# DavidSevic/gpu-nbody-simulation

Measured on AMD Instinct MI355X. Metric: body-steps/sec, higher is better.
Workload: dtype f32

## Files before the change

### gpu-nbody-simulation_amd/csrc/bh_engine.hip

```cpp
#include "../../include/bhgpu.h"

#include <hip/hip_runtime.h>

#include <algorithm>
#include <cmath>
#include <cstdio>
#include <cstdlib>
#include <cstring>
#include <string>
#include <type_traits>
#include <vector>

#include "bh_tree.hpp"
#include "bh_walk_exact.hpp"
#include "bh_walk_f64.hpp"
#include "bh_diag.hpp"
#include "bh_direct.hpp"
#include "bh_field.hpp"
#include "bh_init.hpp"
#include "bh_let.hpp"
#include "bh_migrate.hpp"
#include "bh_split.hpp"
#include "bh_moments.hpp"
#include "bh_radial.hpp"
// ... 28 lines not shown
    double eps = 0.0, eps2 = 0.0;
    float eps2f = 0.f;
    bool exact_thresholds = false;
    int device = 0;
    hipStream_t stream = nullptr;
    bool own_stream = false;
    int64_t n = 0;
    int64_t internal_cap = 0, node_cap = 0;
    int64_t bfs_max = 12288;
    int exact_bpw = 0;
    int walk_split = 0;
    bool walk_asm = true;
    int sort_bucket = 1;
    uint64_t *splitters = nullptr;
    uint16_t *sort_dig = nullptr;
    int build_items = 0;
    bool hilbert = false;
    bool chain_collapse = true;
    double *bslots = nullptr;

    void *pos = nullptr, *vel = nullptr, *mass = nullptr, *force = nullptr;
    void *pos2 = nullptr, *vel2 = nullptr, *mass2 = nullptr, *force2 = nullptr;
    uint32_t *orig = nullptr, *orig2 = nullptr;
    int reorder_every = 16;
    float2 *spos = nullptr;
    float4 *sstate = nullptr;
    float *smass = nullptr;
    uint64_t *keys[2] = {nullptr, nullptr};
    uint32_t *vals[2] = {nullptr, nullptr};
    uint64_t *keys_sorted = nullptr;
// ... 213 lines not shown

void clean_slots(bh_ctx *c) { if (c->carry.slots_dirty) hipLaunchKernelGGL(bounds_slots_reset, dim3(1), dim3(kWave), 0, c->stream, c->bslots); }

template <int SI>
int enqueue_lsd_passes(hipStream_t st, uint64_t *const keys[2], uint32_t *const vals[2], uint32_t *counts, uint32_t *rows, int64_t n,
                       int bits, bool packed)
{
    constexpr int SB = kSortBits;
    const unsigned nbl = blocks_for(n, kBlock * SI);
    const int passes = (bits + SB - 1) / SB;
    int cur = 0;
    for (int p = 0; p < passes; ++p) {
        const int shift = p * SB;
        auto scatter = [&](auto kern) {
            hipLaunchKernelGGL(kern, dim3(nbl), dim3(kBlock), 0, st, keys[cur], packed ? nullptr : vals[cur], keys[cur ^ 1],
                               vals[cur ^ 1], counts, rows, n, shift, (int)nbl, nullptr, nullptr);
        };
        hipLaunchKernelGGL((radix_hist<SI, SB>), dim3(nbl), dim3(kBlock), 0, st, keys[cur], counts, n, shift, (int)nbl);
        hipLaunchKernelGGL(radix_rowscan, dim3(1 << SB), dim3(kBlock), 0, st, counts, rows, (int)nbl);
        if (!packed) scatter(radix_scatter_w<SI, SB>);
        else if (p + 1 == passes) scatter(radix_scatter_w<SI, SB, 2>);
        else scatter(radix_scatter_w<SI, SB, 1>);
        cur ^= 1;
    }
    return cur;
}

template <bool TREE64, bool STATE64 = TREE64, int ITEMS = kItems>
int enqueue_build_t(bh_ctx *c, bool may_reorder, bool time_groups)
{
    constexpr int TILE = kBlock * ITEMS;
// ... 15 lines not shown
            hipLaunchKernelGGL((bounds_partial<Real2>), dim3(nbb), dim3(kBlock), 0, st, pos, n, slots);
        }
    }
    BuildDone done{n, slots != nullptr, false, false, false, false};

    if (n > 0) {
        const bool pack = Dm >= 1 && 2 * Dm <= kPackShift && n <= ((int64_t)1 << (64 - kPackShift))
                          && c->sort_pack;
        const bool single = pack && n >= 2 && n <= 4 * kBsThreads && c->sort_bucket == 1;
        const bool bucket = !single && pack && n >= 2 && n <= kBucketMaxNBig && (c->sort_bucket == 2 || (c->sort_bucket == 1 && c->carry.samples_n == n));
        const int nb = (n <= kBucketMaxN) ? kBuckets : kBucketsBig;
        const int ns = (nb == kBuckets) ? ((n > (int64_t)1 << 18) ? 2 * kBuckets : kBuckets)
                                        : ((n > (int64_t)3 << 20) ? kMaxSplitSamples : kBucketsBig);
        static_assert(kBucketMaxN == (int64_t)1 << 20 && kBucketMaxNBig == (int64_t)1 << 22, "BASELINE configs 3 and 4 fit");
        done.sort_bucket = bucket || single; done.sort_packed = pack;
        {
            const unsigned nkb = blocks_for(n, kBlock);
            auto keys_launch = [&](auto fs, auto pk, auto hil) {
                constexpr bool H = decltype(hil)::value, P = decltype(pk)::value, F = decltype(fs)::value;
                const bool smp = P && bucket;
                hipLaunchKernelGGL((keys_kernel<Real2, H, P, F>), dim3(nkb + (smp ? ns / kWave : 0)), dim3(kBlock), 0, st, pos, c->box,
                                   c->keys[0], c->vals[0], n, Dm, (smp && !TREE64) ? (const float2 *)c->spos : nullptr, c->splitters, nb, ns,
                                   slots, c->ctr, smp ? c->bsum_sort : nullptr, smp ? nb : 0, (smp && TREE64) ? c->perm : nullptr,
                                   from_walk ? 1 : 0);
            };
            dispatch(keys_launch, slots != nullptr, pack, c->hilbert);
        }
        if (time_groups) (void)hipEventRecord(c->ev_grp[0], st);
        const unsigned nbl = blocks_for(n, ITEMS == kItems ? kSortTile : TILE);
        int cur = 0;
        if (single) {
            hipLaunchKernelGGL(bucket_sort_kernel, dim3(1), dim3(kBsThreads), 0, st, c->keys[0], c->keys[1], c->vals[1],
                               nullptr, nullptr, &c->ctr->sort_spills, &c->ctr->sort_reruns, (int)n);
            cur = 1;
        } else if (bucket) {
            constexpr int SI = (ITEMS == kItems ? kSortItems : ITEMS);
            auto pass = [&](auto bits_tag) {
                constexpr int NBITS = decltype(bits_tag)::value;
                if constexpr (TREE64) {
                    hipLaunchKernelGGL((radix_hist<SI, NBITS, true>), dim3(nbl), dim3(kBlock), 0, st, c->keys[0], c->radix_counts, n,
                                       0, (int)nbl, c->splitters, c->sort_dig, nullptr);
                    hipLaunchKernelGGL(radix_rowscan, dim3(1 << NBITS), dim3(kBlock), 0, st, c->radix_counts, c->bsum_sort, (int)nbl);
                    hipLaunchKernelGGL((radix_scatter_w<SI, NBITS, 1, true, false>), dim3(nbl), dim3(kBlock), 0, st, c->keys[0], c->vals[0],
                                       c->keys[1], c->vals[1], c->radix_counts, c->bsum_sort, n, 0, (int)nbl, c->sort_dig,
                                       c->bsum_sort + kBucketStartOffset);
                } else {
                    hipLaunchKernelGGL((radix_hist<SI, NBITS, true>), dim3(nbl), dim3(kBlock), 0, st, c->keys[0], c->radix_counts, n,
                                       0, (int)nbl, c->splitters, c->sort_dig, c->bsum_sort);
                    hipLaunchKernelGGL((radix_scatter_w<SI, NBITS, 1, true>), dim3(nbl), dim3(kBlock), 0, st, c->keys[0], c->vals[0],
                                       c->keys[1], c->vals[1], c->radix_counts, c->bsum_sort, n, 0, (int)nbl, c->sort_dig,
                                       c->bsum_sort + kBucketStartOffset);
                }
            };
            if (nb == kBuckets) pass(std::integral_constant<int, 8>{}); else pass(std::integral_constant<int, 10>{});
            hipLaunchKernelGGL(bucket_sort_kernel, dim3(nb), dim3(kBsThreads), 0, st, c->keys[1], c->keys[0], c->vals[0],
                               c->bsum_sort, c->bsum_sort + kBucketStartOffset, &c->ctr->sort_spills, &c->ctr->sort_reruns, 0);
            cur = 0;
        } else {
            constexpr int SI = (ITEMS == kItems ? kSortItems : ITEMS);
            cur = enqueue_lsd_passes<SI>(st, c->keys, c->vals, c->radix_counts, c->bsum_sort, n, 2 * Dm, pack);
        }
        c->keys_sorted = c->keys[cur];
        c->perm = c->vals[cur];
        if constexpr (!TREE64) {
            if (may_reorder && c->reorder_every > 0 && c->carry.builds % c->reorder_every == 0) {
                hipLaunchKernelGGL((reorder_state_kernel<Real2, Real>), dim3(blocks_for(n, kBlock)), dim3(kBlock), 0, st,
                                   c->perm, pos, static_cast<const Real2 *>(c->vel), mass,
                                   static_cast<const float2 *>(c->force), c->is.orig_identity ? nullptr : c->orig,
                                   static_cast<Real2 *>(c->pos2), static_cast<Real2 *>(c->vel2),
                                   static_cast<Real *>(c->mass2), static_cast<float2 *>(c->force2), c->orig2, n);
                std::swap(c->pos, c->pos2); std::swap(c->vel, c->vel2); std::swap(c->mass, c->mass2);
                std::swap(c->force, c->force2); std::swap(c->orig, c->orig2);
// ... 388 lines not shown
    bh_ctx *c = new bh_ctx();
    c->cfg = *cfg;
    c->Dm = cfg->max_depth - 1;
    c->mode = cfg->precision == BH_PRECISION_F64_EXACT ? Mode::Exact
            : cfg->precision == BH_PRECISION_F64       ? Mode::F64
            : cfg->precision == BH_PRECISION_MIXED     ? Mode::Mixed : Mode::F32;
    c->compat = cfg->reference_compat != 0;
    c->device = cfg->device;
    if (const char *e = std::getenv("BH_WALK_SPLIT")) c->walk_split = std::atoi(e);
    if (const char *e = std::getenv("BH_EXACT_BPW")) { const int b = std::atoi(e); c->exact_bpw = (b >= 1 && b <= kWave && (b & (b - 1)) == 0) ? b : 0; }
    if (const char *e = std::getenv("BH_WALK_ASM")) c->walk_asm = std::atoi(e) != 0;
    if (const char *e = std::getenv("BH_EXACT_BFS_MAX")) c->bfs_max = std::max(0, std::atoi(e));
    c->exact_thresholds = c->mode == Mode::Exact && c->walk_asm && !(cfg->flags & BH_FLAG_WALK_PORTABLE);
    if (const char *e = std::getenv("BH_SORT_PACK")) c->sort_pack = std::atoi(e) != 0;
    if (const char *e = std::getenv("BH_SORT_BUCKET")) c->sort_bucket = std::atoi(e);
    if (const char *e = std::getenv("BH_BUILD_ITEMS")) c->build_items = std::atoi(e);
    if (const char *e = std::getenv("BH_REORDER_EVERY")) c->reorder_every = std::max(0, std::atoi(e));
    c->hilbert = !c->tree64();
    if (const char *e = std::getenv("BH_HILBERT")) c->hilbert = !c->tree64() && std::atoi(e) != 0;
    if (const char *e = std::getenv("BH_CHAIN_COLLAPSE")) c->chain_collapse = std::atoi(e) != 0;
    if (const char *e = std::getenv("BH_RADIAL_BLOCKS")) { const int b = std::atoi(e); if (b >= 1 && b <= 65536) c->rad_blocks = b; }
    auto bail = [&](int rc) { g_create_error = c->err; bh_destroy(c); return rc; };

    if (hipSetDevice(c->device) != hipSuccess) { c->err = "hipSetDevice failed"; return bail(BH_ERR_DEVICE); }
    if (hipStreamCreateWithFlags(&c->stream, hipStreamNonBlocking) != hipSuccess) {
        c->err = "hipStreamCreate failed"; return bail(BH_ERR_DEVICE);
    }
    c->own_stream = true;

    const int64_t cap = std::max<int64_t>(cfg->capacity, 1);
// ... 15 lines not shown
    if (!c->tree64()) {
        { char *t; A(&t, cap * 2 * rs); c->pos2 = t; }
        { char *t; A(&t, cap * 2 * rs); c->vel2 = t; }
        { char *t; A(&t, cap * rs); c->mass2 = t; }
        { char *t; A(&t, cap * 2 * sizeof(float)); c->force2 = t; }
        A(&c->orig, cap); A(&c->orig2, cap);
    }
    A(&c->keys[0], cap); A(&c->keys[1], cap); A(&c->vals[0], cap); A(&c->vals[1], cap);
    A(&c->cnt, cap + 1);
    { const size_t nbl = std::max<size_t>(blocks_for(cap, kSortTile), blocks_for(std::min<int64_t>(cap, 1 << 22), kBlock * kSmallItems));
      const size_t big = (cap > kBucketMaxN) ? (size_t)kBucketsBig * blocks_for(std::min<int64_t>(cap, kBucketMaxNBig), kBlock * kSmallItems) : 0;
      A(&c->radix_counts, std::max<size_t>((size_t)(1 << kSortBits) * nbl, big));
      A(&c->bsum_sort, 2 * kBucketStartOffset);
      A(&c->splitters, kBucketsBig);
      A(&c->sort_dig, (size_t)std::min<int64_t>(cap, kBucketMaxNBig) + 16);
    }
    const size_t scan_tiles = std::max<size_t>(blocks_for(cap + 1, kTile), blocks_for(std::min<int64_t>(cap, 1 << 22) + 1, kBlock * kSmallItems)) + 8;
    A(&c->bsum_u32, scan_tiles);
    A(&c->partial, 4 * (std::max<size_t>(1024, blocks_for(cap, kWave)) + 2));
    A(&c->box, 8); A(&c->bslots, 4 * kBoundSlots);
    A(&c->ctr, 1);
    if (c->tree64()) {
        { NodeD *g0 = nullptr; LinkD *l0 = nullptr; A(&g0, c->node_cap + 4); A(&l0, c->node_cap + 4);
          if (!rc) { c->gd = g0 + 3; c->ld = l0 + 3; } }
        A(&c->self_node, c->internal_cap + 1); A(&c->com_pending, c->internal_cap + 1); A(&c->cell_depth, c->internal_cap + 1);
        A(&c->cell_first, c->internal_cap + 1);
    } else {
        A(&c->qf, c->internal_cap + 1); A(&c->aux, 4 * (c->internal_cap + 1));
        A(&c->cell_first, c->internal_cap + 1);
        A(&c->gid, cap); A(&c->group_cost, cap / kWave + 2); A(&c->walk_consts, 4);
        A(&c->coarse, cap / 256 + 2);
        A(&c->spos, cap); A(&c->sstate, cap + 64 * kBlock + 1024); A(&c->smass, cap);
        A(&c->terms, cap + 1); A(&c->bsum_d3, scan_tiles);
    }
    if (rc) return bail(rc);
    if (hipMemset(c->ctr, 0, sizeof(TreeCounters)) != hipSuccess) { c->err = "hipMemset failed"; return bail(BH_ERR_DEVICE); }
    if (!c->tree64()) {
        const void *wc[4] = {c->aux, c->spos, c->smass, nullptr};
        if (hipMemcpy(c->walk_consts, wc, sizeof(wc), hipMemcpyHostToDevice) != hipSuccess) { c->err = "hipMemcpy failed"; return bail(BH_ERR_DEVICE); }
    }
    if (!c->tree64() && c->exp.create(cap) != hipSuccess) { c->err = "experiment hooks: allocation failed"; return bail(BH_ERR_DEVICE); }
    auto create = [](auto &evs) { for (auto &e : evs) if (hipEventCreate(&e) != hipSuccess) return false; return true; };
    if (!create(c->ev_step) || !create(c->ev_build) || !create(c->ev_grp) || !create(c->ev_let)) {
        c->err = "hipEventCreate failed"; return bail(BH_ERR_DEVICE);
    }
    *out = c;
    return BH_OK;
}

void bh_destroy(bh_ctx *c)
{
// ... 2235 lines not shown
```

### gpu-nbody-simulation_amd/csrc/bh_sort.hpp

```cpp
#pragma once

#include "bh_prims.hpp"

namespace bh {

#ifndef BH_SORT_ITEMS
#define BH_SORT_ITEMS 8
#endif
constexpr int kSortItems = BH_SORT_ITEMS;
constexpr int kSortTile = kBlock * kSortItems;
constexpr int kRadixBits = 8;

__global__ __launch_bounds__(kBlock) void radix_rowscan(uint32_t *__restrict__ counts,
                                                         uint32_t *__restrict__ row_total, int nblocks)
{
    __shared__ uint32_t sm[kWavesPerBlock + 1];
    uint32_t *row = counts + (int64_t)blockIdx.x * nblocks;
    uint32_t carry = 0;
    for (int c0 = 0; c0 < nblocks; c0 += kBlock) {
        const int b = c0 + threadIdx.x;
        const uint32_t v = (b < nblocks) ? row[b] : 0u;
        uint32_t tot;
        const uint32_t ex = block_exclusive_sum(v, sm, tot);
        if (b < nblocks) row[b] = carry + ex;
// ... 8 lines not shown
constexpr int kSortBits = 8;
constexpr int kBuckets = 256, kBucketsBig = 1024;
constexpr int kBucketStartOffset = kBucketsBig + 8;
constexpr int kDigits = 256;
constexpr int kMaxSplitSamples = 2048;
constexpr uint64_t kKeyMask40 = (1ull << 40) - 1;
template <int NB>
__device__ __forceinline__ uint32_t bucket_of(uint64_t key, const uint64_t *spl)
{
    int b = 0;
#pragma unroll
    for (int s = NB / 2; s >= 1; s >>= 1) b += (spl[b + s] <= key) ? s : 0;
    return (uint32_t)b;
}

__device__ __forceinline__ bool wave_same_digit(uint32_t d, bool valid)
{
    return __ballot(valid) == ~0ull && __ballot(d != (uint32_t)__builtin_amdgcn_readfirstlane((int)d)) == 0ull;
}
template <bool TRY = true>
__device__ __forceinline__ void wave_count_digit(uint32_t *row, uint32_t d, bool valid)
{
    if (TRY && wave_same_digit(d, valid)) {
        if (lane_id() == 0) atomicAdd(&row[d], (uint32_t)kWave);
    } else if (valid) {
        atomicAdd(&row[d], 1u);
    }
}

template <int ITEMS, int BITS = kRadixBits, bool BUCKET = false>
__global__ __launch_bounds__(kBlock) void radix_hist(const uint64_t *__restrict__ keys,
                                                      uint32_t *__restrict__ counts, int64_t n,
                                                      int shift, int nblocks,
                                                      const uint64_t *__restrict__ splitters = nullptr,
                                                      uint16_t *__restrict__ dig16 = nullptr,
                                                      uint32_t *__restrict__ row_total = nullptr)
{
    constexpr int R = 1 << BITS;
    __shared__ uint32_t h[R];
    __shared__ uint64_t spl[BUCKET ? R : 1];
    if (BUCKET)
        for (int d = threadIdx.x; d < R; d += kBlock) {
            const uint64_t v = splitters[d];
            spl[d] = (d > 0 && splitters[d - 1] == v) ? v + 1 : v;
        }
    for (int d = threadIdx.x; d < R; d += kBlock) h[d] = 0;
    __syncthreads();
    const int64_t base = (int64_t)blockIdx.x * (kBlock * ITEMS);
    uint32_t guess = 0;
#pragma unroll
    for (int r = 0; r < ITEMS; ++r) {
        const int64_t i = base + r * kBlock + threadIdx.x;
        const bool valid = i < n;
        const uint64_t k = valid ? keys[i] : 0ull;
        uint32_t d;
        if (BUCKET) {
            const uint64_t kk = k & kKeyMask40;
            bool ok = false;
            if (r > 0) ok = spl[guess] <= kk && (guess + 1 == (uint32_t)R || kk < spl[guess + 1]);
            if (r > 0 && __ballot(valid && !ok) == 0ull) d = guess;
            else d = bucket_of<R>(kk, spl);
            guess = d;
// ... 11 lines not shown
    }
}


constexpr int kPackShift = 40;
constexpr uint64_t kPackKeyMask = (1ull << kPackShift) - 1;
template <int ITEMS, int BITS = kRadixBits, int PACK = 0, bool BUCKET = false, bool RAW = BUCKET>
__global__ __launch_bounds__(kBlock) void radix_scatter_w(const uint64_t *__restrict__ kin,
                                                           const uint32_t *__restrict__ vin,
                                                           uint64_t *__restrict__ kout,
                                                           uint32_t *__restrict__ vout,
                                                           const uint32_t *__restrict__ offs,
                                                           const uint32_t *__restrict__ row_total, int64_t n,
                                                           int shift, int nblocks,
                                                           const uint16_t *__restrict__ dig16 = nullptr,
                                                           uint32_t *__restrict__ bucket_start = nullptr)
{
    static_assert(!BUCKET || PACK == 1, "the bucket pass moves packed keys");
    constexpr int TILE = kBlock * ITEMS;
    constexpr int R = 1 << BITS, DPT = R / kBlock;
    static_assert(R % kBlock == 0, "whole digits per thread");
    __shared__ uint32_t woff[kWavesPerBlock][R];
    __shared__ int32_t gdelta[R];
    __shared__ uint64_t skey[TILE];
    __shared__ uint32_t sval[PACK ? 1 : TILE];
    __shared__ uint32_t sm[kWavesPerBlock + 1];
    __shared__ uint16_t sdig[BUCKET ? TILE : 1];
    __shared__ uint64_t match[kWavesPerBlock][R];
    constexpr int kRowsTogether = 64;
    __shared__ uint32_t s_np, s_plist[kRowsTogether], s_before[kRowsTogether];
    const int t = threadIdx.x, w = wave_id(), l = lane_id();
    for (int d = t; d < R; d += kBlock)
#pragma unroll
        for (int k = 0; k < kWavesPerBlock; ++k) { woff[k][d] = 0; match[k][d] = 0ull; }
    __syncthreads();

    const int64_t tile_base = (int64_t)blockIdx.x * TILE;
    const int64_t base = tile_base + (int64_t)w * (kWave * ITEMS);
    uint64_t key[ITEMS];
    uint32_t val[PACK ? 1 : ITEMS];
    uint32_t dig[ITEMS], rank[ITEMS], npeer[ITEMS];
#pragma unroll
    for (int r = 0; r < ITEMS; ++r) {
        const int64_t i = base + r * kWave + l;
        const bool valid = i < n;
        key[r] = valid ? kin[i] : ~0ull;
        if (!PACK) val[r] = valid ? vin[i] : 0u;
        dig[r] = BUCKET ? (valid ? (uint32_t)dig16[i] : 0u) : (uint32_t)(key[r] >> shift) & (R - 1);
    }
#pragma unroll
// ... 143 lines not shown
{
    const int w = wave_id();
    const uint32_t inc = wave_inclusive_sum(v);
    if (w < 4 && lane_id() == kWave - 1) sm[w] = inc;
    __syncthreads();
    uint32_t base = 0, tot = 0;
#pragma unroll
    for (int k = 0; k < 4; ++k) { const uint32_t q = sm[k]; base += (k < w) ? q : 0u; tot += q; }
    __syncthreads();
    total = tot;
    return base + inc - v;
}

constexpr int kFixRun = 8;
template <int ITEMS>
__device__ __forceinline__ void bucket_sort_lds(const uint64_t *__restrict__ in, int m, uint64_t *skey,
                                                uint32_t (*woff)[kDigits], uint64_t (*match)[kDigits],
                                                uint32_t *sm, uint64_t *s_red, uint32_t *s_flag,
                                                uint64_t *__restrict__ kout, uint32_t *__restrict__ vout,
                                                uint32_t *__restrict__ reruns)
{
    const int t = threadIdx.x, w = wave_id(), l = lane_id();
    const int wbase = w * (kWave * ITEMS);
    uint64_t key[ITEMS];
    uint64_t kmin = ~0ull, kmax = 0ull;
#pragma unroll
    for (int r = 0; r < ITEMS; ++r) {
        const int i = wbase + r * kWave + l;
        key[r] = (i < m) ? in[i] : ~0ull;
        if (i < m) {
            const uint64_t k = key[r] & kKeyMask40;
// ... 111 lines not shown
                    if ((q >> first) != top) break;
                    delta += ((q & lowmask) < low) ? 1 : 0;
                }
                too_long = too_long || (j < m && j - i > kFixRun);
                kout[i + delta] = kk + kmin;
                vout[i + delta] = (uint32_t)(word >> kPackShift);
            }
        }
        if (too_long) *s_flag = 1u;
        __syncthreads();
        if (*s_flag == 0u) return;
        if (t == 0) atomicAdd(reruns, 1u);
#pragma unroll
        for (int r = 0; r < ITEMS; ++r) {
            const int i = wbase + r * kWave + l;
            key[r] = (i < m) ? in[i] - kmin : ~0ull;
        }
        for (int k = t; k < kBsWaves * kDigits; k += kBsThreads) (&woff[0][0])[k] = 0;
        __syncthreads();
        first = 0; passes = full; fix = false;
    }
    for (int i = t; i < m; i += kBsThreads) {
        const uint64_t k = skey[i];
        kout[i] = (k & kKeyMask40) + kmin;
        vout[i] = (uint32_t)(k >> kPackShift);
    }
}

__global__ __launch_bounds__(kBsThreads) void bucket_sort_kernel(uint64_t *__restrict__ bucketed,
                                                                  uint64_t *__restrict__ kout,
                                                                  uint32_t *__restrict__ vout,
                                                                  const uint32_t *__restrict__ bucket_total,
                                                                  const uint32_t *__restrict__ bucket_start,
                                                                  uint32_t *__restrict__ spills,
                                                                  uint32_t *__restrict__ reruns, int single_m)
{
    __shared__ uint64_t skey[kBucketCap];
    __shared__ uint32_t woff[kBsWaves][kDigits];
    __shared__ uint64_t match[kBsWaves][kDigits];
    __shared__ uint32_t sm[8];
    __shared__ uint64_t s_or[2 * kBsWaves];
    __shared__ uint32_t s_flag;
    const int t = threadIdx.x, w = wave_id(), l = lane_id();
    const int64_t start = bucket_total ? (int64_t)bucket_start[blockIdx.x] : 0;
    const int m = bucket_total ? (int)bucket_total[blockIdx.x] : single_m;
    if (m == 0) return;
    uint64_t *in = bucketed + start;
    uint64_t *ko = kout + start;
    uint32_t *vo = vout + start;

    if (m <= 1 * kBsThreads) { bucket_sort_lds<1>(in, m, skey, woff, match, sm, s_or, &s_flag, ko, vo, reruns); return; }
    if (m <= 2 * kBsThreads) { bucket_sort_lds<2>(in, m, skey, woff, match, sm, s_or, &s_flag, ko, vo, reruns); return; }
    if (m <= 4 * kBsThreads) { bucket_sort_lds<4>(in, m, skey, woff, match, sm, s_or, &s_flag, ko, vo, reruns); return; }
    if (m <= 5 * kBsThreads) { bucket_sort_lds<5>(in, m, skey, woff, match, sm, s_or, &s_flag, ko, vo, reruns); return; }
    if (m <= 6 * kBsThreads) { bucket_sort_lds<6>(in, m, skey, woff, match, sm, s_or, &s_flag, ko, vo, reruns); return; }
    if (m <= 8 * kBsThreads) { bucket_sort_lds<8>(in, m, skey, woff, match, sm, s_or, &s_flag, ko, vo, reruns); return; }
    if (m <= kBucketCap) { bucket_sort_lds<kBucketItemsMax>(in, m, skey, woff, match, sm, s_or, &s_flag, ko, vo, reruns); return; }

    const uint64_t k0 = in[0];
    uint64_t x = 0;
    for (int i = t; i < m; i += kBsThreads) x |= (in[i] ^ k0) & kKeyMask40;
#pragma unroll
// ... 70 lines not shown
```

### gpu-nbody-simulation_amd/csrc/bh_tree.hpp

```cpp
#pragma once

#include <type_traits>

#include "bh_prims.hpp"
#include "bh_sort.hpp"
#include "bh_nodes.hpp"
#include "bh_bounds.hpp"

namespace bh {

constexpr int kCoarse = 256;

__device__ __forceinline__ int shared_levels(uint64_t a, uint64_t b, int Dm)
{
    const uint64_t x = a ^ b;
    if (x == 0) return Dm;
    return (__clzll((long long)x) - (64 - 2 * Dm)) >> 1;
}

template <typename Real2>
__global__ __launch_bounds__(kBlock) void bounds_partial(const Real2 *__restrict__ pos, int64_t n, double *slots)
{
    double xlo = INFINITY, xhi = -INFINITY, ylo = INFINITY, yhi = -INFINITY;
    for (int64_t i = (int64_t)blockIdx.x * kBlock + threadIdx.x; i < n; i += (int64_t)gridDim.x * kBlock) {
// ... 65 lines not shown
__device__ __forceinline__ uint32_t hilbert3_entry(uint32_t t)
{
    int state = (int)(t >> 6);
    const uint32_t iy3 = (t >> 3) & 7u, ix3 = t & 7u;
    uint32_t digits = 0;
#pragma unroll
    for (int l = 2; l >= 0; --l) {
        const int c = (int)(((ix3 >> l) & 1u) | (((iy3 >> l) & 1u) << 1));
        digits = (digits << 2) | (uint32_t)hilbert_digit(state, c);
        state = hilbert_next(state, c);
    }
    return ((uint32_t)state << 6) | digits;
}

template <bool HILBERT>
__device__ __forceinline__ uint64_t key_of_fast(double x, double y, double x0, double x1, double y0, double y1, int Dm,
                                                double scale_x, double scale_y, double margin_x, double margin_y,
                                                const uint8_t *hil3 = nullptr)
{
    const double side = (double)(1u << Dm);
    const double tx = (x - x0) * scale_x, ty = (y - y0) * scale_y;
    const double fx = floor(tx), fy = floor(ty);
    const double rx = tx - fx, ry = ty - fy;
    const bool sure = rx > margin_x && rx < 1.0 - margin_x && ry > margin_y && ry < 1.0 - margin_y &&
                      fx >= 0.0 && fx < side && fy >= 0.0 && fy < side;
    if (!sure) return key_of<HILBERT>(x, y, x0, x1, y0, y1, Dm);
    const uint32_t ix = (uint32_t)fx, iy = (uint32_t)fy;
    uint64_t k = 0;
    int state = 0;
    int l = Dm - 1;
    if (HILBERT && hil3 != nullptr) {
        for (; (l + 1) % 3 != 0; --l) {
            const int c = (int)(((ix >> l) & 1u) | (((iy >> l) & 1u) << 1));
            k = (k << 2) | (uint64_t)hilbert_digit(state, c);
            state = hilbert_next(state, c);
        }
        uint32_t st = (uint32_t)state;
        for (; l >= 2; l -= 3) {
            const uint32_t e = hil3[(st << 6) | (((iy >> (l - 2)) & 7u) << 3) | ((ix >> (l - 2)) & 7u)];
            k = (k << 6) | (uint64_t)(e & 63u);
            st = e >> 6;
        }
// ... 7 lines not shown
            u = (u | (u << 4)) & 0x0F0F0F0F0F0F0F0Full;
            u = (u | (u << 2)) & 0x3333333333333333ull;
            u = (u | (u << 1)) & 0x5555555555555555ull;
            return u;
        };
        return spread(ix) | (spread(iy) << 1);
    }
    for (; l >= 0; --l) {
        const int c = (int)(((ix >> l) & 1u) | (((iy >> l) & 1u) << 1));
        k = (k << 2) | (uint64_t)hilbert_digit(state, c);
        state = hilbert_next(state, c);
    }
    return k;
}

template <typename Real2, bool HILBERT, bool PACK = false, bool FROM_SLOTS = false>
__global__ __launch_bounds__(kBlock) void keys_kernel(const Real2 *__restrict__ pos,
                                                       double *box_global,
                                                       uint64_t *__restrict__ keys,
                                                       uint32_t *__restrict__ idx, int64_t n, int Dm,
                                                       const float2 *__restrict__ samples = nullptr,
                                                       uint64_t *__restrict__ splitters = nullptr, int nb = 0,
                                                       int ns = 0, double *slots = nullptr, TreeCounters *ctr = nullptr,
                                                       uint32_t *__restrict__ zero_words = nullptr, int n_zero = 0,
                                                       const uint32_t *__restrict__ sample_perm = nullptr, int from_walk = 0)
{
    if (blockIdx.x == 0)
        for (int k = threadIdx.x; k < n_zero; k += kBlock) zero_words[k] = 0u;
    __shared__ double s_box[FROM_SLOTS ? 8 : 1];
    __shared__ int s_keep;
    if (FROM_SLOTS) {
        if (threadIdx.x < kWave) {
            const double *sl = slots + 4 * threadIdx.x;
            const double xlo = wave_min(sl[0]), xhi = wave_max(sl[1]), ylo = wave_min(sl[2]), yhi = wave_max(sl[3]);
            const bool keep = from_walk && xlo > xhi;
            if (threadIdx.x == 0) s_keep = keep ? 1 : 0;
            if (threadIdx.x < 2) {
                const int a = threadIdx.x;
                if (keep) {
                    s_box[2 * a] = box_global[2 * a]; s_box[2 * a + 1] = box_global[2 * a + 1];
                    s_box[4 + a] = box_global[4 + a]; s_box[6 + a] = box_global[6 + a];
                } else {
                    const double ex = xhi - xlo, ey = yhi - ylo;
// ... 12 lines not shown
                for (int k = 0; k < 8; ++k) box_global[k] = s_box[k];
                ctr->overflow = 0;
            }
            ctr->n_internal = 0;
            ctr->visits = 0; ctr->interactions = 0; ctr->wave_nodes = 0; ctr->wave_quads = 0; ctr->wave_accepts = 0;
        }
    }
    double x0, x1, y0, y1, bk4, bk5, bk6, bk7;
    if (FROM_SLOTS) {
        x0 = s_box[0]; x1 = s_box[1]; y0 = s_box[2]; y1 = s_box[3]; bk4 = s_box[4]; bk5 = s_box[5]; bk6 = s_box[6]; bk7 = s_box[7];
    } else {
        x0 = box_global[0]; x1 = box_global[1]; y0 = box_global[2]; y1 = box_global[3];
        bk4 = box_global[4]; bk5 = box_global[5]; bk6 = box_global[6]; bk7 = box_global[7];
    }
    const int nsb = (samples != nullptr || sample_perm != nullptr) ? ns / kWave : 0;
    if ((int)blockIdx.x < nsb) {
        __shared__ uint64_t sk[kMaxSplitSamples];
        const int t = threadIdx.x;
        const int Ds = Dm, lg_ns = 31 - __clz(ns), lg_os = lg_ns - (31 - __clz(nb));
        const double side = (double)(1u << Ds), top = side - 1.0, down = 1.0 / (double)(1u << (Dm - Ds));
        const double sx = (bk4 > 0.0) ? bk4 * down : side / (x1 - x0), sy = (bk5 > 0.0) ? bk5 * down : side / (y1 - y0);
        float2 qs[kMaxSplitSamples / kBlock];
#pragma unroll
        for (int k = 0; k < kMaxSplitSamples / kBlock; ++k) {
            const int j = t + k * kBlock;
            qs[k] = float2{0.f, 0.f};
            if (j < ns) {
                const int64_t rk = ((int64_t)j * n) >> lg_ns;
                if (sample_perm != nullptr) { const Real2 pp = pos[sample_perm[rk]]; qs[k] = float2{(float)pp.x, (float)pp.y}; }
                else qs[k] = samples[rk];
            }
        }
#pragma unroll
// ... 14 lines not shown
                }
            }
            sk[j] = (mine << 11) | (uint64_t)j;
        }
        __syncthreads();
        const int sidx = (int)blockIdx.x * kWave + (t >> 2), part = t & 3, span = ns >> 2;
        const uint64_t tagged = sk[sidx];
        int rank = 0;
#pragma unroll 16
        for (int q = part * span; q < (part + 1) * span; ++q) rank += (sk[q] < tagged) ? 1 : 0;
        rank += __shfl_xor(rank, 1);
        rank += __shfl_xor(rank, 2);
        if (part == 0 && (rank & ((1 << lg_os) - 1)) == 0) splitters[rank >> lg_os] = tagged >> 11;
        return;
    }
    __shared__ uint8_t s_hil3[HILBERT ? 256 : 1];
    if (HILBERT) {
        static_assert(kBlock == 256, "one table entry per thread");
        s_hil3[threadIdx.x] = (uint8_t)hilbert3_entry(threadIdx.x);
        __syncthreads();
    }
    const int64_t i = ((int64_t)blockIdx.x - nsb) * kBlock + threadIdx.x;
    if (i >= n) return;
    const uint64_t k = key_of_fast<HILBERT>((double)pos[i].x, (double)pos[i].y, x0, x1, y0, y1, Dm, bk4, bk5, bk6, bk7,
                                            HILBERT ? s_hil3 : nullptr);
    if (PACK) {
        keys[i] = k | ((uint64_t)i << kPackShift);
    } else {
        keys[i] = k;
        idx[i] = (uint32_t)i;
    }
}

template <bool EXACT, int ITEMS, typename Real2, typename Real, typename SReal2 = Real2, typename SReal = Real>
__global__ __launch_bounds__(kBlock) void prep_kernel(const uint64_t *__restrict__ keys,
                                                       const uint32_t *__restrict__ perm,
                                                       const Real2 *__restrict__ pos,
                                                       const Real *__restrict__ mass,
                                                       uint32_t *__restrict__ cnt,
                                                       uint32_t *__restrict__ bsum_u32,
                                                       SReal2 *__restrict__ spos, SReal *__restrict__ smass,
                                                       d3 *__restrict__ terms, d3 *__restrict__ bsum_d3,
// ... 808 lines not shown
```

Before: 2.420 billion.

## Skip bucket radix pass when few bodies change bucket since last sort

When the sample set is unchanged, the keys kernel checks each body's new key against the key range of its previous bucket slot (fixed-length ranges over the prior sorted order). Bodies that leave their range are appended to per-wave sub-lists through atomics. If the total stays under a small cap, the radix histogram and scatter kernels exit early, and the bucket sort kernel rebuilds each bucket from the previous order plus the crossing list. This adds counters, scratch buffers, double-buffered counter slots and overflow fallbacks, and risks extra work whenever many bodies move.

```diff
diff --git a/gpu-nbody-simulation_amd/csrc/bh_engine.hip b/gpu-nbody-simulation_amd/csrc/bh_engine.hip
--- a/gpu-nbody-simulation_amd/csrc/bh_engine.hip
+++ b/gpu-nbody-simulation_amd/csrc/bh_engine.hip
@@ -66,6 +66,14 @@
     int sort_bucket = 1;
     uint64_t *splitters = nullptr;
     uint16_t *sort_dig = nullptr;
+    int sort_direct = 1;
+    int64_t sort_direct_max = kSortDirectMax;
+    uint64_t *keys_scatter = nullptr;
+    uint64_t *direct_list = nullptr, *direct_range_keys = nullptr;
+    uint32_t *direct_count = nullptr;
+    uint32_t direct_cap = 0, direct_subcap = 0;
+    int direct_nsub = 1;
+    int direct_slot = 0;
     int build_items = 0;
     bool hilbert = false;
     bool chain_collapse = true;
@@ -309,7 +317,7 @@
         const int shift = p * SB;
         auto scatter = [&](auto kern) {
             hipLaunchKernelGGL(kern, dim3(nbl), dim3(kBlock), 0, st, keys[cur], packed ? nullptr : vals[cur], keys[cur ^ 1],
-                               vals[cur ^ 1], counts, rows, n, shift, (int)nbl, nullptr, nullptr);
+                               vals[cur ^ 1], counts, rows, n, shift, (int)nbl, nullptr, nullptr, nullptr, 0u, 0u, 1);
         };
         hipLaunchKernelGGL((radix_hist<SI, SB>), dim3(nbl), dim3(kBlock), 0, st, keys[cur], counts, n, shift, (int)nbl);
         hipLaunchKernelGGL(radix_rowscan, dim3(1 << SB), dim3(kBlock), 0, st, counts, rows, (int)nbl);
@@ -355,6 +363,19 @@
                                         : ((n > (int64_t)3 << 20) ? kMaxSplitSamples : kBucketsBig);
         static_assert(kBucketMaxN == (int64_t)1 << 20 && kBucketMaxNBig == (int64_t)1 << 22, "BASELINE configs 3 and 4 fit");
         done.sort_bucket = bucket || single; done.sort_packed = pack;
+        const bool direct = bucket && !TREE64 && c->sort_direct != 0 && c->carry.samples_n == n;
+        SortDirect sd;
+        BucketDirect bd;
+        if (direct) {
+            const uint32_t len = (uint32_t)((n + nb - 1) / nb);
+            sd.count = c->direct_count + c->direct_slot * kDirectCounterWords;
+            sd.count_next = c->direct_count + (c->direct_slot ^ 1) * kDirectCounterWords;
+            sd.list = c->direct_list; sd.range_keys = c->direct_range_keys; sd.cap = c->direct_cap; sd.subcap = c->direct_subcap;
+            sd.len = len; sd.nsub = c->direct_nsub;
+            bd.count = sd.count; bd.list = sd.list; bd.range_keys = sd.range_keys; bd.keys = c->keys[0]; bd.scratch = c->keys_scatter;
+            bd.n = n; bd.cap = sd.cap; bd.subcap = sd.subcap; bd.len = len; bd.nb = nb; bd.nsub = sd.nsub;
+            c->direct_slot ^= 1;
+        }
         {
             const unsigned nkb = blocks_for(n, kBlock);
             auto keys_launch = [&](auto fs, auto pk, auto hil) {
@@ -363,7 +384,7 @@
                 hipLaunchKernelGGL((keys_kernel<Real2, H, P, F>), dim3(nkb + (smp ? ns / kWave : 0)), dim3(kBlock), 0, st, pos, c->box,
                                    c->keys[0], c->vals[0], n, Dm, (smp && !TREE64) ? (const float2 *)c->spos : nullptr, c->splitters, nb, ns,
                                    slots, c->ctr, smp ? c->bsum_sort : nullptr, smp ? nb : 0, (smp && TREE64) ? c->perm : nullptr,
-                                   from_walk ? 1 : 0);
+                                   from_walk ? 1 : 0, smp ? sd : SortDirect{});
             };
             dispatch(keys_launch, slots != nullptr, pack, c->hilbert);
         }
@@ -372,7 +393,7 @@
         int cur = 0;
         if (single) {
             hipLaunchKernelGGL(bucket_sort_kernel, dim3(1), dim3(kBsThreads), 0, st, c->keys[0], c->keys[1], c->vals[1],
-                               nullptr, nullptr, &c->ctr->sort_spills, &c->ctr->sort_reruns, (int)n);
+                               nullptr, nullptr, &c->ctr->sort_spills, &c->ctr->sort_reruns, (int)n, BucketDirect{});
             cur = 1;
         } else if (bucket) {
             constexpr int SI = (ITEMS == kItems ? kSortItems : ITEMS);
@@ -387,16 +408,23 @@
                                        c->bsum_sort + kBucketStartOffset);
                 } else {
                     hipLaunchKernelGGL((radix_hist<SI, NBITS, true>), dim3(nbl), dim3(kBlock), 0, st, c->keys[0], c->radix_counts, n,
-                                       0, (int)nbl, c->splitters, c->sort_dig, c->bsum_sort);
+                                       0, (int)nbl, c->splitters, c->sort_dig, c->bsum_sort, sd.count, sd.cap, sd.subcap, sd.nsub);
                     hipLaunchKernelGGL((radix_scatter_w<SI, NBITS, 1, true>), dim3(nbl), dim3(kBlock), 0, st, c->keys[0], c->vals[0],
-                                       c->keys[1], c->vals[1], c->radix_counts, c->bsum_sort, n, 0, (int)nbl, c->sort_dig,
-                                       c->bsum_sort + kBucketStartOffset);
+                                       direct ? c->keys_scatter : c->keys[1], c->vals[1], c->radix_counts, c->bsum_sort, n, 0, (int)nbl,
+                                       c->sort_dig, c->bsum_sort + kBucketStartOffset, sd.count, sd.cap, sd.subcap, sd.nsub);
                 }
             };
             if (nb == kBuckets) pass(std::integral_constant<int, 8>{}); else pass(std::integral_constant<int, 10>{});
-            hipLaunchKernelGGL(bucket_sort_kernel, dim3(nb), dim3(kBsThreads), 0, st, c->keys[1], c->keys[0], c->vals[0],
-                               c->bsum_sort, c->bsum_sort + kBucketStartOffset, &c->ctr->sort_spills, &c->ctr->sort_reruns, 0);
-            cur = 0;
+            if (direct) {
+                hipLaunchKernelGGL(bucket_sort_kernel, dim3(nb), dim3(kBsThreads), 0, st, c->keys_scatter, c->keys[1], c->vals[1],
+                                   c->bsum_sort, c->bsum_sort + kBucketStartOffset, &c->ctr->sort_spills, &c->ctr->sort_reruns, 0, bd);
+                cur = 1;
+            } else {
+                hipLaunchKernelGGL(bucket_sort_kernel, dim3(nb), dim3(kBsThreads), 0, st, c->keys[1], c->keys[0], c->vals[0],
+                                   c->bsum_sort, c->bsum_sort + kBucketStartOffset, &c->ctr->sort_spills, &c->ctr->sort_reruns, 0,
+                                   BucketDirect{});
+                cur = 0;
+            }
         } else {
             constexpr int SI = (ITEMS == kItems ? kSortItems : ITEMS);
             cur = enqueue_lsd_passes<SI>(st, c->keys, c->vals, c->radix_counts, c->bsum_sort, n, 2 * Dm, pack);
@@ -815,6 +843,9 @@
     c->exact_thresholds = c->mode == Mode::Exact && c->walk_asm && !(cfg->flags & BH_FLAG_WALK_PORTABLE);
     if (const char *e = std::getenv("BH_SORT_PACK")) c->sort_pack = std::atoi(e) != 0;
     if (const char *e = std::getenv("BH_SORT_BUCKET")) c->sort_bucket = std::atoi(e);
+    if (const char *e = std::getenv("BH_SORT_DIRECT")) { const int d = std::atoi(e); c->sort_direct = (d >= 0 && d <= 2) ? d : 1; }
+    if (const char *e = std::getenv("BH_SORT_DIRECT_MAX")) c->sort_direct_max = std::max<long long>(0, std::atoll(e));
+    if (c->tree64()) c->sort_direct = 0;
     if (const char *e = std::getenv("BH_BUILD_ITEMS")) c->build_items = std::atoi(e);
     if (const char *e = std::getenv("BH_REORDER_EVERY")) c->reorder_every = std::max(0, std::atoi(e));
     c->hilbert = !c->tree64();
@@ -860,6 +891,17 @@
       A(&c->bsum_sort, 2 * kBucketStartOffset);
       A(&c->splitters, kBucketsBig);
       A(&c->sort_dig, (size_t)std::min<int64_t>(cap, kBucketMaxNBig) + 16);
+      if (c->sort_direct) {
+          const int64_t most = std::min<int64_t>(cap, kBucketMaxNBig);
+          c->direct_cap = (uint32_t)std::min<int64_t>(most, c->sort_direct == 2 ? most : c->sort_direct_max);
+          c->direct_nsub = c->sort_direct == 2 ? 1 : kDirectSubs;
+          c->direct_subcap = c->direct_cap;
+          if (c->sort_direct != 2) { c->direct_subcap = 16; while ((int64_t)c->direct_subcap * (kDirectSubs / 4) < c->direct_cap) c->direct_subcap *= 2; }
+          A(&c->keys_scatter, (size_t)most);
+          A(&c->direct_list, std::max<size_t>((size_t)c->direct_nsub * c->direct_subcap, 1));
+          A(&c->direct_range_keys, kBucketsBig);
+          A(&c->direct_count, 2 * kDirectCounterWords);
+      }
     }
     const size_t scan_tiles = std::max<size_t>(blocks_for(cap + 1, kTile), blocks_for(std::min<int64_t>(cap, 1 << 22) + 1, kBlock * kSmallItems)) + 8;
     A(&c->bsum_u32, scan_tiles);
@@ -881,6 +923,7 @@
     }
     if (rc) return bail(rc);
     if (hipMemset(c->ctr, 0, sizeof(TreeCounters)) != hipSuccess) { c->err = "hipMemset failed"; return bail(BH_ERR_DEVICE); }
+    if (c->direct_count && hipMemset(c->direct_count, 0, 2 * kDirectCounterWords * sizeof(uint32_t)) != hipSuccess) { c->err = "hipMemset failed"; return bail(BH_ERR_DEVICE); }
     if (!c->tree64()) {
         const void *wc[4] = {c->aux, c->spos, c->smass, nullptr};
         if (hipMemcpy(c->walk_consts, wc, sizeof(wc), hipMemcpyHostToDevice) != hipSuccess) { c->err = "hipMemcpy failed"; return bail(BH_ERR_DEVICE); }
diff --git a/gpu-nbody-simulation_amd/csrc/bh_sort.hpp b/gpu-nbody-simulation_amd/csrc/bh_sort.hpp
--- a/gpu-nbody-simulation_amd/csrc/bh_sort.hpp
+++ b/gpu-nbody-simulation_amd/csrc/bh_sort.hpp
@@ -46,6 +46,49 @@
     return (uint32_t)b;
 }
 
+__device__ __forceinline__ uint32_t bucket_of_n(uint64_t key, const uint64_t *spl, int nb)
+{
+    int b = 0;
+    for (int s = nb >> 1; s >= 1; s >>= 1) b += (spl[b + s] <= key) ? s : 0;
+    return (uint32_t)b;
+}
+
+constexpr int64_t kSortDirectMax = 1024;
+constexpr int kDirectSubs = 64;
+constexpr int kDirectCounterWords = 64 * (1 + kDirectSubs);
+constexpr uint32_t kDirectStride = 64;
+constexpr uint64_t kRangeKeyInf = ~0ull;
+struct SortDirect {
+    uint32_t *count = nullptr;
+    uint32_t *count_next = nullptr;
+    uint64_t *list = nullptr;
+    uint64_t *range_keys = nullptr;
+    uint32_t cap = 0;
+    uint32_t subcap = 0;
+    uint32_t len = 0;
+    int nsub = 1;
+};
+struct DirectWords { uint32_t v, off; };
+__device__ __forceinline__ DirectWords direct_load(const uint32_t *count, int nsub)
+{
+    const int l = threadIdx.x & 63;
+    return DirectWords{(l < nsub) ? count[kDirectStride * (1u + (uint32_t)l)] : 0u, count[0]};
+}
+__device__ __forceinline__ uint32_t direct_total(DirectWords w, uint32_t cap, uint32_t subcap)
+{
+    const uint32_t v = w.v, off = w.off;
+    uint32_t total = v;
+#pragma unroll
+    for (int o = 32; o >= 1; o >>= 1) total += (uint32_t)__shfl_xor((int)total, o);
+    const bool bad = off != 0u || __ballot(v > subcap) != 0ull || total > cap;
+    return bad ? ~0u : total;
+}
+__device__ __forceinline__ uint32_t direct_total(const uint32_t *count, int nsub, uint32_t cap, uint32_t subcap)
+{
+    return direct_total(direct_load(count, nsub), cap, subcap);
+}
+__device__ __forceinline__ bool stays_in(uint64_t key40, uint64_t lo, uint64_t hi) { return lo <= key40 && key40 < hi; }
+
 __device__ __forceinline__ bool wave_same_digit(uint32_t d, bool valid)
 {
     return __ballot(valid) == ~0ull && __ballot(d != (uint32_t)__builtin_amdgcn_readfirstlane((int)d)) == 0ull;
@@ -66,8 +109,12 @@
                                                       int shift, int nblocks,
                                                       const uint64_t *__restrict__ splitters = nullptr,
                                                       uint16_t *__restrict__ dig16 = nullptr,
-                                                      uint32_t *__restrict__ row_total = nullptr)
-{
+                                                      uint32_t *__restrict__ row_total = nullptr,
+                                                      const uint32_t *__restrict__ direct_count = nullptr,
+                                                      uint32_t direct_cap = 0, uint32_t direct_subcap = 0, int direct_nsub = 1)
+{
+    DirectWords dw{0u, 1u};
+    if (BUCKET && direct_count != nullptr) dw = direct_load(direct_count, direct_nsub);
     constexpr int R = 1 << BITS;
     __shared__ uint32_t h[R];
     __shared__ uint64_t spl[BUCKET ? R : 1];
@@ -78,6 +125,7 @@
         }
     for (int d = threadIdx.x; d < R; d += kBlock) h[d] = 0;
     __syncthreads();
+    if (BUCKET && direct_count != nullptr && direct_total(dw, direct_cap, direct_subcap) != ~0u) return;
     const int64_t base = (int64_t)blockIdx.x * (kBlock * ITEMS);
     uint32_t guess = 0;
 #pragma unroll
@@ -119,9 +167,13 @@
                                                            const uint32_t *__restrict__ row_total, int64_t n,
                                                            int shift, int nblocks,
                                                            const uint16_t *__restrict__ dig16 = nullptr,
-                                                           uint32_t *__restrict__ bucket_start = nullptr)
+                                                           uint32_t *__restrict__ bucket_start = nullptr,
+                                                           const uint32_t *__restrict__ direct_count = nullptr,
+                                                           uint32_t direct_cap = 0, uint32_t direct_subcap = 0, int direct_nsub = 1)
 {
     static_assert(!BUCKET || PACK == 1, "the bucket pass moves packed keys");
+    DirectWords dw{0u, 1u};
+    if (BUCKET && direct_count != nullptr) dw = direct_load(direct_count, direct_nsub);
     constexpr int TILE = kBlock * ITEMS;
     constexpr int R = 1 << BITS, DPT = R / kBlock;
     static_assert(R % kBlock == 0, "whole digits per thread");
@@ -139,6 +191,7 @@
 #pragma unroll
         for (int k = 0; k < kWavesPerBlock; ++k) { woff[k][d] = 0; match[k][d] = 0ull; }
     __syncthreads();
+    if (BUCKET && direct_count != nullptr && direct_total(dw, direct_cap, direct_subcap) != ~0u) return;
 
     const int64_t tile_base = (int64_t)blockIdx.x * TILE;
     const int64_t base = tile_base + (int64_t)w * (kWave * ITEMS);
@@ -312,7 +365,7 @@
 
 constexpr int kFixRun = 8;
 template <int ITEMS>
-__device__ __forceinline__ void bucket_sort_lds(const uint64_t *__restrict__ in, int m, uint64_t *skey,
+__device__ __forceinline__ void bucket_sort_lds(const uint64_t *in, int m, uint64_t *skey,
                                                 uint32_t (*woff)[kDigits], uint64_t (*match)[kDigits],
                                                 uint32_t *sm, uint64_t *s_red, uint32_t *s_flag,
                                                 uint64_t *__restrict__ kout, uint32_t *__restrict__ vout,
@@ -454,8 +507,9 @@
 #pragma unroll
         for (int r = 0; r < ITEMS; ++r) {
             const int i = wbase + r * kWave + l;
-            key[r] = (i < m) ? in[i] - kmin : ~0ull;
-        }
+            key[r] = (i < m) ? skey[i] : ~0ull;
+        }
+        __syncthreads();
         for (int k = t; k < kBsWaves * kDigits; k += kBsThreads) (&woff[0][0])[k] = 0;
         __syncthreads();
         first = 0; passes = full; fix = false;
@@ -465,6 +519,32 @@
         kout[i] = (k & kKeyMask40) + kmin;
         vout[i] = (uint32_t)(k >> kPackShift);
     }
+}
+
+struct BucketDirect {
+    const uint32_t *count = nullptr;
+    const uint64_t *list = nullptr;
+    const uint64_t *range_keys = nullptr;
+    uint64_t *keys = nullptr;
+    uint64_t *scratch = nullptr;
+    int64_t n = 0;
+    uint32_t cap = 0, subcap = 0, len = 0;
+    int nb = 0, nsub = 1;
+};
+constexpr int kDirectItems = 4;
+constexpr int kMineCap = kBsWaves * kDigits - kBucketsBig;
+
+__device__ __forceinline__ uint32_t bs_sum1024(uint32_t v, uint32_t *tmp, uint32_t &exclusive)
+{
+    const uint32_t inc = wave_inclusive_sum(v);
+    if (lane_id() == kWave - 1) tmp[wave_id()] = inc;
+    __syncthreads();
+    uint32_t base = 0, tot = 0;
+#pragma unroll
+    for (int k = 0; k < kBsWaves; ++k) { const uint32_t q = tmp[k]; base += (k < wave_id()) ? q : 0u; tot += q; }
+    __syncthreads();
+    exclusive = base + inc - v;
+    return tot;
 }
 
 __global__ __launch_bounds__(kBsThreads) void bucket_sort_kernel(uint64_t *__restrict__ bucketed,
@@ -473,7 +553,8 @@
                                                                   const uint32_t *__restrict__ bucket_total,
                                                                   const uint32_t *__restrict__ bucket_start,
                                                                   uint32_t *__restrict__ spills,
-                                                                  uint32_t *__restrict__ reruns, int single_m)
+                                                                  uint32_t *__restrict__ reruns, int single_m,
+                                                                  BucketDirect dz = BucketDirect{})
 {
     __shared__ uint64_t skey[kBucketCap];
     __shared__ uint32_t woff[kBsWaves][kDigits];
@@ -481,11 +562,111 @@
     __shared__ uint32_t sm[8];
     __shared__ uint64_t s_or[2 * kBsWaves];
     __shared__ uint32_t s_flag;
+    __shared__ uint32_t s_dz[3];
     const int t = threadIdx.x, w = wave_id(), l = lane_id();
-    const int64_t start = bucket_total ? (int64_t)bucket_start[blockIdx.x] : 0;
-    const int m = bucket_total ? (int)bucket_total[blockIdx.x] : single_m;
-    if (m == 0) return;
-    uint64_t *in = bucketed + start;
+    int64_t start;
+    int m;
+    uint64_t *in;
+    const int64_t counted_start = bucket_total ? (int64_t)bucket_start[blockIdx.x] : 0;
+    const int counted_m = bucket_total ? (int)bucket_total[blockIdx.x] : single_m;
+    const uint32_t crossers = dz.count ? direct_total(dz.count, dz.nsub, dz.cap, dz.subcap) : ~0u;
+    if (crossers == ~0u) {
+        start = counted_start;
+        m = counted_m;
+        if (m == 0) return;
+        in = bucketed + start;
+    } else {
+        const int b = (int)blockIdx.x;
+        const int64_t r0 = ((int64_t)b * dz.len < dz.n) ? (int64_t)b * dz.len : dz.n;
+        const int len = (int)((r0 + dz.len < dz.n ? r0 + dz.len : dz.n) - r0);
+        if (crossers == 0u) {
+            start = r0; m = len;
+            if (m == 0) return;
+            in = dz.keys + r0;
+        } else {
+            uint64_t *spl = &match[0][0];
+            uint64_t *mine = spl + kBucketsBig;
+            uint32_t *delta = &woff[0][0];
+            uint32_t *held = reinterpret_cast<uint32_t *>(skey);
+            for (int k = t; k < dz.nb; k += kBsThreads) { spl[k] = dz.range_keys[k]; delta[k] = 0u; }
+            if (t < 3) s_dz[t] = 0u;
+            if (t < dz.nsub) held[t] = dz.count[kDirectStride * (1u + (uint32_t)t)];
+            __syncthreads();
+            uint32_t most = 0;
+            for (int k = 0; k < dz.nsub; ++k) most = (held[k] > most) ? held[k] : most;
+            const uint32_t slots = (dz.nsub > 1) ? (uint32_t)dz.nsub * dz.subcap : most;
+            const uint32_t lg_sub = 31u - (uint32_t)__clz(dz.nsub > 1 ? (int)dz.subcap : 1);
+            auto listed = [&](uint32_t x) -> bool { return dz.nsub > 1 ? (x & (dz.subcap - 1u)) < held[x >> lg_sub] : true; };
+            for (uint32_t e = (uint32_t)t; e < slots; e += kBsThreads) {
+                if (!listed(e)) continue;
+                const uint64_t word = dz.list[e];
+                const uint32_t idx = (uint32_t)(word >> kPackShift);
+                const int dst = (int)bucket_of_n(word & kKeyMask40, spl, dz.nb), src = (int)(idx / dz.len);
+                atomicAdd(&delta[dst], 1u);
+                atomicSub(&delta[src], 1u);
+                if (dst == b) {
+                    const uint32_t k = atomicAdd(&s_dz[0], 1u);
+                    if (k < (uint32_t)kMineCap) mine[k] = word;
+                    if ((int64_t)idx < r0) atomicAdd(&s_dz[1], 1u);
+                }
+                if (src == b) atomicAdd(&s_dz[2], 1u);
+            }
+            __syncthreads();
+            uint32_t part = 0, ex;
+            for (int k = t; k < b; k += kBsThreads) part += delta[k];
+            uint32_t *tmp = reinterpret_cast<uint32_t *>(s_or);
+            const uint32_t moved = bs_sum1024(part, tmp, ex);
+            const uint32_t arrived = s_dz[0], lower = s_dz[1], left = s_dz[2];
+            start = r0 + (int64_t)(int32_t)moved;
+            m = len - (int)left + (int)arrived;
+            if (m <= 0 || start < 0 || start + m > dz.n) return;
+            if (arrived == 0u && left == 0u) {
+                in = dz.keys + r0;
+            } else {
+                uint64_t *ko_ = kout + start;
+                const uint64_t *arr = mine;
+                if (arrived > (uint32_t)kMineCap) {
+                    __syncthreads();
+                    if (t == 0) s_dz[0] = 0u;
+                    __syncthreads();
+                    for (uint32_t e = (uint32_t)t; e < slots; e += kBsThreads) {
+                        if (!listed(e)) continue;
+                        const uint64_t word = dz.list[e];
+                        if ((int)bucket_of_n(word & kKeyMask40, spl, dz.nb) == b) ko_[atomicAdd(&s_dz[0], 1u)] = word;
+                    }
+                    __threadfence_block();
+                    __syncthreads();
+                    arr = ko_;
+                }
+                uint64_t *g = (m <= kBucketCap) ? skey : dz.scratch + start;
+                const uint64_t lo = spl[b], hi = (b + 1 < dz.nb) ? spl[b + 1] : kRangeKeyInf;
+                uint64_t own[kDirectItems];
+                uint32_t c = 0;
+#pragma unroll
+                for (int j = 0; j < kDirectItems; ++j) {
+                    const int i = kDirectItems * t + j;
+                    own[j] = (i < len) ? dz.keys[r0 + i] : kRangeKeyInf;
+                    c += (i < len && stays_in(own[j] & kKeyMask40, lo, hi)) ? 1u : 0u;
+                }
+                const uint32_t stay = bs_sum1024(c, tmp, ex);
+                uint32_t o = lower + ex;
+#pragma unroll
+                for (int j = 0; j < kDirectItems; ++j)
+                    if (kDirectItems * t + j < len && stays_in(own[j] & kKeyMask40, lo, hi)) { if (o < (uint32_t)m) g[o] = own[j]; ++o; }
+                for (uint32_t q = (uint32_t)t; q < arrived; q += kBsThreads) {
+                    const uint64_t word = arr[q];
+                    const uint32_t idx = (uint32_t)(word >> kPackShift);
+                    uint32_t rank = 0;
+                    for (uint32_t r = 0; r < arrived; ++r) rank += ((uint32_t)(arr[r] >> kPackShift) < idx) ? 1u : 0u;
+                    const uint32_t slot = rank + (((int64_t)idx < r0) ? 0u : stay);
+                    if (slot < (uint32_t)m) g[slot] = word;
+                }
+                __threadfence_block();
+                __syncthreads();
+                in = g;
+            }
+        }
+    }
     uint64_t *ko = kout + start;
     uint32_t *vo = vout + start;
 
diff --git a/gpu-nbody-simulation_amd/csrc/bh_tree.hpp b/gpu-nbody-simulation_amd/csrc/bh_tree.hpp
--- a/gpu-nbody-simulation_amd/csrc/bh_tree.hpp
+++ b/gpu-nbody-simulation_amd/csrc/bh_tree.hpp
@@ -103,18 +103,8 @@
 }
 
 template <bool HILBERT>
-__device__ __forceinline__ uint64_t key_of_fast(double x, double y, double x0, double x1, double y0, double y1, int Dm,
-                                                double scale_x, double scale_y, double margin_x, double margin_y,
-                                                const uint8_t *hil3 = nullptr)
-{
-    const double side = (double)(1u << Dm);
-    const double tx = (x - x0) * scale_x, ty = (y - y0) * scale_y;
-    const double fx = floor(tx), fy = floor(ty);
-    const double rx = tx - fx, ry = ty - fy;
-    const bool sure = rx > margin_x && rx < 1.0 - margin_x && ry > margin_y && ry < 1.0 - margin_y &&
-                      fx >= 0.0 && fx < side && fy >= 0.0 && fy < side;
-    if (!sure) return key_of<HILBERT>(x, y, x0, x1, y0, y1, Dm);
-    const uint32_t ix = (uint32_t)fx, iy = (uint32_t)fy;
+__device__ __forceinline__ uint64_t curve_key(uint32_t ix, uint32_t iy, int Dm, const uint8_t *hil3 = nullptr)
+{
     uint64_t k = 0;
     int state = 0;
     int l = Dm - 1;
@@ -152,6 +142,21 @@
     return k;
 }
 
+template <bool HILBERT>
+__device__ __forceinline__ uint64_t key_of_fast(double x, double y, double x0, double x1, double y0, double y1, int Dm,
+                                                double scale_x, double scale_y, double margin_x, double margin_y,
+                                                const uint8_t *hil3 = nullptr)
+{
+    const double side = (double)(1u << Dm);
+    const double tx = (x - x0) * scale_x, ty = (y - y0) * scale_y;
+    const double fx = floor(tx), fy = floor(ty);
+    const double rx = tx - fx, ry = ty - fy;
+    const bool sure = rx > margin_x && rx < 1.0 - margin_x && ry > margin_y && ry < 1.0 - margin_y &&
+                      fx >= 0.0 && fx < side && fy >= 0.0 && fy < side;
+    if (!sure) return key_of<HILBERT>(x, y, x0, x1, y0, y1, Dm);
+    return curve_key<HILBERT>((uint32_t)fx, (uint32_t)fy, Dm, hil3);
+}
+
 template <typename Real2, bool HILBERT, bool PACK = false, bool FROM_SLOTS = false>
 __global__ __launch_bounds__(kBlock) void keys_kernel(const Real2 *__restrict__ pos,
                                                        double *box_global,
@@ -161,10 +166,14 @@
                                                        uint64_t *__restrict__ splitters = nullptr, int nb = 0,
                                                        int ns = 0, double *slots = nullptr, TreeCounters *ctr = nullptr,
                                                        uint32_t *__restrict__ zero_words = nullptr, int n_zero = 0,
-                                                       const uint32_t *__restrict__ sample_perm = nullptr, int from_walk = 0)
-{
-    if (blockIdx.x == 0)
+                                                       const uint32_t *__restrict__ sample_perm = nullptr, int from_walk = 0,
+                                                       SortDirect sd = SortDirect{})
+{
+    if (blockIdx.x == 0) {
         for (int k = threadIdx.x; k < n_zero; k += kBlock) zero_words[k] = 0u;
+        if (sd.count_next != nullptr)
+            for (int k = threadIdx.x; k <= sd.nsub; k += kBlock) sd.count_next[kDirectStride * k] = 0u;
+    }
     __shared__ double s_box[FROM_SLOTS ? 8 : 1];
     __shared__ int s_keep;
     if (FROM_SLOTS) {
@@ -207,9 +216,37 @@
         bk4 = box_global[4]; bk5 = box_global[5]; bk6 = box_global[6]; bk7 = box_global[7];
     }
     const int nsb = (samples != nullptr || sample_perm != nullptr) ? ns / kWave : 0;
+    __shared__ uint8_t s_hil3[HILBERT ? 256 : 1];
+    if (HILBERT) {
+        static_assert(kBlock == 256, "one table entry per thread");
+        s_hil3[threadIdx.x] = (uint8_t)hilbert3_entry(threadIdx.x);
+        __syncthreads();
+    }
+    const bool direct = PACK && sd.count != nullptr;
+    auto range_has_body = [&](uint32_t j) -> bool { return j > 0u && j < (uint32_t)nb && (int64_t)j * sd.len < n; };
+    auto range_key_at = [&](uint32_t j, bool has_body, Real2 pp) -> uint64_t {
+        if (!has_body) return (j == 0u) ? 0ull : kRangeKeyInf;
+        const double side = (double)(1u << Dm), top = side - 1.0;
+        const double sx = (bk4 > 0.0) ? bk4 : side / (x1 - x0), sy = (bk5 > 0.0) ? bk5 : side / (y1 - y0);
+        const double fx = fmin(fmax(((double)pp.x - x0) * sx, 0.0), top);
+        const double fy = fmin(fmax(((double)pp.y - y0) * sy, 0.0), top);
+        return curve_key<HILBERT>((uint32_t)(int)fx, (uint32_t)(int)fy, Dm, HILBERT ? s_hil3 : nullptr);
+    };
+    auto range_key = [&](uint32_t j) -> uint64_t {
+        const bool has_body = range_has_body(j);
+        return range_key_at(j, has_body, has_body ? pos[(int64_t)j * sd.len] : Real2{});
+    };
     if ((int)blockIdx.x < nsb) {
         __shared__ uint64_t sk[kMaxSplitSamples];
         const int t = threadIdx.x;
+        if (direct && blockIdx.x == 0) {
+            for (int j = t; j < nb; j += kBlock) { const uint64_t v = range_key((uint32_t)j); sk[j] = v; sd.range_keys[j] = v; }
+            __syncthreads();
+            int bad = 0;
+            for (int j = t; j + 1 < nb; j += kBlock) bad |= (sk[j] > sk[j + 1]) ? 1 : 0;
+            bad = __syncthreads_or(bad);
+            if (bad && t == 0) sd.count[0] = 1u;
+        }
         const int Ds = Dm, lg_ns = 31 - __clz(ns), lg_os = lg_ns - (31 - __clz(nb));
         const double side = (double)(1u << Ds), top = side - 1.0, down = 1.0 / (double)(1u << (Dm - Ds));
         const double sx = (bk4 > 0.0) ? bk4 * down : side / (x1 - x0), sy = (bk5 > 0.0) ? bk5 * down : side / (y1 - y0);
@@ -254,18 +291,56 @@
         if (part == 0 && (rank & ((1 << lg_os) - 1)) == 0) splitters[rank >> lg_os] = tagged >> 11;
         return;
     }
-    __shared__ uint8_t s_hil3[HILBERT ? 256 : 1];
-    if (HILBERT) {
-        static_assert(kBlock == 256, "one table entry per thread");
-        s_hil3[threadIdx.x] = (uint8_t)hilbert3_entry(threadIdx.x);
+    const int64_t i0 = ((int64_t)blockIdx.x - nsb) * kBlock;
+    const int64_t i = i0 + threadIdx.x;
+    __shared__ uint64_t s_rk[kBlock + 2];
+    uint32_t b0 = 0, need = 0;
+    Real2 range_pos{};
+    bool range_body = false;
+    if (direct) {
+        b0 = (uint32_t)i0 / sd.len;
+        const int64_t last = ((i0 + kBlock < n) ? i0 + kBlock : n) - 1;
+        need = (uint32_t)last / sd.len - b0 + 1u;
+        range_body = threadIdx.x <= need && range_has_body(b0 + threadIdx.x);
+        if (range_body) range_pos = pos[(int64_t)(b0 + threadIdx.x) * sd.len];
+    } else if (i >= n) {
+        return;
+    }
+    uint64_t k = 0;
+    if (i < n) k = key_of_fast<HILBERT>((double)pos[i].x, (double)pos[i].y, x0, x1, y0, y1, Dm, bk4, bk5, bk6, bk7,
+                                        HILBERT ? s_hil3 : nullptr);
+    if (direct) {
+        if (threadIdx.x <= need) s_rk[threadIdx.x] = range_key_at(b0 + threadIdx.x, range_body, range_pos);
+        if (need == (uint32_t)kBlock && threadIdx.x == 0) s_rk[kBlock] = range_key(b0 + kBlock);
         __syncthreads();
-    }
-    const int64_t i = ((int64_t)blockIdx.x - nsb) * kBlock + threadIdx.x;
-    if (i >= n) return;
-    const uint64_t k = key_of_fast<HILBERT>((double)pos[i].x, (double)pos[i].y, x0, x1, y0, y1, Dm, bk4, bk5, bk6, bk7,
-                                            HILBERT ? s_hil3 : nullptr);
+        if (i >= n) return;
+    }
     if (PACK) {
-        keys[i] = k | ((uint64_t)i << kPackShift);
+        const uint64_t word = k | ((uint64_t)i << kPackShift);
+        keys[i] = word;
+        if (direct) {
+            const uint32_t off = (uint32_t)(i - (int64_t)b0 * sd.len);
+            uint32_t q = (uint32_t)((float)off * (1.0f / (float)sd.len));
+            if (q * sd.len > off) --q; else if ((q + 1u) * sd.len <= off) ++q;
+            const bool cross = !stays_in(k, s_rk[q], s_rk[q + 1u]);
+            const uint64_t who = __ballot(cross);
+            if (who != 0ull) {
+                const uint32_t mine = (uint32_t)__popcll(who);
+                const uint32_t sub = ((uint32_t)(i0 >> 6) + (uint32_t)wave_id()) & (uint32_t)(sd.nsub - 1);
+                uint32_t *ctr = sd.count + kDirectStride * (1u + sub);
+                const int leader = __ffsll((unsigned long long)who) - 1;
+                uint32_t base = ~0u;
+                if (lane_id() == leader && mine <= (uint32_t)kWave / 2u && sd.count[0] == 0u &&
+                    __hip_atomic_load(ctr, __ATOMIC_RELAXED, __HIP_MEMORY_SCOPE_AGENT) <= sd.subcap)
+                    base = atomicAdd(ctr, mine);
+                base = (uint32_t)__shfl((int)base, leader);
+                if (base == ~0u || base + mine > sd.subcap) {
+                    if (lane_id() == leader && sd.count[0] == 0u) sd.count[0] = 1u;
+                } else if (cross) {
+                    sd.list[(size_t)sub * sd.subcap + base + (uint32_t)__popcll(who & ((1ull << lane_id()) - 1ull))] = word;
+                }
+            }
+        }
     } else {
         keys[i] = k;
         idx[i] = (uint32_t)i;
```

Result: faster. 2.475 billion, median of 6 (+2.3%).
